# EPOCHDevs/PandasArrow

Hardware: AMD Instinct MI355X
Metric: Grows/sec hash group-by-sum, 1e9 int64 rows x 1e6 keys (higher is better)
Workload: dtype f64; 1 GPU; group_by(int64 key).agg(sum,mean,count), 1e+09 rows / 1e+06 keys, 1 GPU; rows=1000000000, keys=1000000, rows_per_gpu=1000000000, parity=bit-exact vs Arrow-order pairwise sum

## Files before the change

pandasarrow_amd/csrc/gb_flr_reduce.hpp:

```cpp
#pragma once

constexpr int kFlrBits = 6;
constexpr int kFlrLevels = 20;
#ifndef PDX_FLR_ITEMS
#define PDX_FLR_ITEMS 10
#endif
#ifndef PDX_FLR_DENSE_WAVES
#define PDX_FLR_DENSE_WAVES 1
#endif
#ifndef PDX_FLR_BATCH_RANK
#define PDX_FLR_BATCH_RANK 1
#endif
#ifndef PDX_FLR_DPP_SCAN
#define PDX_FLR_DPP_SCAN 1
#endif
constexpr bool kFlrDppScan = PDX_FLR_DPP_SCAN != 0;
#ifndef PDX_FLR_RANK_GROUP
#define PDX_FLR_RANK_GROUP 2
#endif
constexpr int kFlrRankGroup = PDX_FLR_RANK_GROUP;
constexpr bool kFlrBatchRank = PDX_FLR_BATCH_RANK != 0;
constexpr int kFlrDenseWaves = PDX_FLR_DENSE_WAVES;
constexpr int kFlrItems = PDX_FLR_ITEMS;
constexpr int kFlrTile = kSortBlock * kFlrItems;
#ifdef PDX_FLR_TIMING
__device__ unsigned long long g_flr_cycles[2][12];
#define FLR_T(slot)                                                                                     \
  do {                                                                                                  \
    if (DENSE_PW && wave < 2) {                                                                         \
      const unsigned long long now_ = __builtin_readcyclecounter();                                     \
      tacc_[slot] += now_ - tmark_;                                                                     \
      tmark_ = now_;                                                                                    \
    }                                                                                                   \
  } while (0)
#else
#define FLR_T(slot) do { } while (0)
#endif
constexpr int kFlrMaxLeaves = kFlrTile / 16 + ((1 << kFlrBits) * 30) / 16;
constexpr int kFlrLeafStride = kFlrMaxLeaves + 1;
constexpr int kFlrDenseLevels = 16;
__global__ void k_run_starts(const uint32_t* __restrict__ sorted_keys, int64_t n, int low_bits, int64_t nruns, uint32_t* __restrict__ run_start,
                             unsigned int* __restrict__ max_len) {
  const uint32_t lmask = (1u << low_bits) - 1u;
  const int64_t stride = (int64_t)gridDim.x * blockDim.x;
  for (int64_t r = (int64_t)blockIdx.x * blockDim.x + threadIdx.x; r <= nruns; r += stride) {
    int64_t lo = 0, hi = n;
    if (r < nruns) {
      while (lo < hi) {
        int64_t mid = (lo + hi) >> 1;
        if ((int64_t)(sorted_keys[mid] & lmask) < r) lo = mid + 1;
        else hi = mid;
      }
    } else {
      lo = n;
    }
    run_start[r] = (uint32_t)lo;
  }
  (void)max_len;
}
__global__ void k_run_max_len(const uint32_t* __restrict__ run_start, int64_t nruns, unsigned int* __restrict__ out, unsigned int limit) {
  const int64_t stride = (int64_t)gridDim.x * blockDim.x;
  unsigned int m = 0, nl = 0, rl = 0;
  for (int64_t r = (int64_t)blockIdx.x * blockDim.x + threadIdx.x; r < nruns; r += stride) {
    unsigned int len = run_start[r + 1] - run_start[r];
    m = len > m ? len : m;
    if (len > limit) {
      ++nl;
      rl += len;
    }
  }
  for (int d = 32; d >= 1; d >>= 1) {
    unsigned int o = __shfl_xor(m, d, 64);
    m = o > m ? o : m;
// ... 62 lines not shown
    int lo = 0, hi = nl - 1;
    while (lo < hi) {
      const int mid = (lo + hi + 1) >> 1;
      if ((int64_t)soff[mid] <= t) lo = mid;
      else hi = mid - 1;
    }
    const int64_t src = (int64_t)sstart[lo] + (t - (int64_t)soff[lo]);
    const uint32_t k = keys[src];
    uint32_t slot;
    if (sizeof(KT) == 1) slot = (((k & ((1u << kFlrBits) - 1u)) << low_bits) | srun[lo]) | ((k >> 7) << 31);
    else slot = k;
    side_key[t] = slot;
    side_val[t] = vals[src];
  }
}
__device__ __forceinline__ double flr_sqdev(double v, double mu) {
  const double x = v - mu;
  return v != v ? v : (mu != mu ? mu : x * x);
}
__device__ __forceinline__ void flr_counter_push(double (*csum)[1 << kFlrBits], int lane, unsigned long long& cmask, int& root, double leaf) {
  int cur = 0;
  unsigned long long m = 1;
  double v = pw_merge(csum[0][lane], leaf);
  cmask ^= m;
  while ((cmask & m) == 0) {
    csum[cur][lane] = 0.0;
    ++cur;
    m <<= 1;
    v = pw_merge(csum[cur][lane], v);
    cmask ^= m;
  }
  csum[cur][lane] = v;
  root = cur > root ? cur : root;
}
}
#include "flr_wave.hpp"
namespace pdx {
template <int ITEMS, int GROUP>
__device__ __forceinline__ void wave_match_rank_batch(unsigned long long* M, uint32_t* cnt, const uint32_t (&d)[ITEMS], int rows_wave, int lane, uint64_t lt_mask,
                                                      uint32_t (&rank)[ITEMS]) {
#pragma unroll
  for (int q = 0; q < ITEMS; ++q) __hip_atomic_store(&M[q * 64 + lane], 0ull, __ATOMIC_RELAXED, __HIP_MEMORY_SCOPE_WAVEFRONT);
  __builtin_amdgcn_fence(__ATOMIC_ACQ_REL, "wavefront");
#pragma unroll
  for (int q = 0; q < ITEMS; ++q)
    if (q * 64 + lane < rows_wave) __hip_atomic_fetch_or(&M[q * 64 + d[q]], 1ull << lane, __ATOMIC_RELAXED, __HIP_MEMORY_SCOPE_WAVEFRONT);
  __builtin_amdgcn_fence(__ATOMIC_ACQ_REL, "wavefront");
  uint32_t tot = 0;
#pragma unroll
  for (int q0 = 0; q0 < ITEMS; q0 += GROUP) {
    unsigned long long peers[GROUP], own[GROUP];
#pragma unroll
    for (int g = 0; g < GROUP; ++g)
      if (q0 + g < ITEMS) peers[g] = __hip_atomic_load(&M[(q0 + g) * 64 + d[q0 + g]], __ATOMIC_RELAXED, __HIP_MEMORY_SCOPE_WAVEFRONT);
#pragma unroll
    for (int g = 0; g < GROUP; ++g)
      if (q0 + g < ITEMS) own[g] = __hip_atomic_load(&M[(q0 + g) * 64 + lane], __ATOMIC_RELAXED, __HIP_MEMORY_SCOPE_WAVEFRONT);
#pragma unroll
    for (int g = 0; g < GROUP; ++g)
      if (q0 + g < ITEMS) {
        rank[q0 + g] = (uint32_t)__popcll(peers[g] & lt_mask) + (uint32_t)__shfl((int)tot, (int)d[q0 + g], 64);
        tot += (uint32_t)__popcll(own[g]);
      }
  }
  __hip_atomic_store(&cnt[lane], tot, __ATOMIC_RELAXED, __HIP_MEMORY_SCOPE_WAVEFRONT);
  __builtin_amdgcn_fence(__ATOMIC_ACQ_REL, "wavefront");
}
__device__ __forceinline__ uint32_t wave_inclusive_sum_dpp(uint32_t x) {
  x += (uint32_t)__builtin_amdgcn_update_dpp(0, (int)x, 0x111, 0xF, 0xF, true);
  x += (uint32_t)__builtin_amdgcn_update_dpp(0, (int)x, 0x112, 0xF, 0xF, true);
  x += (uint32_t)__builtin_amdgcn_update_dpp(0, (int)x, 0x114, 0xF, 0xF, true);
  x += (uint32_t)__builtin_amdgcn_update_dpp(0, (int)x, 0x118, 0xF, 0xF, true);
  x += (uint32_t)__builtin_amdgcn_update_dpp(0, (int)x, 0x142, 0xA, 0xF, false);
  x += (uint32_t)__builtin_amdgcn_update_dpp(0, (int)x, 0x143, 0xC, 0xF, false);
  return x;
}
struct RunStateOp {
  template <typename U>
  __device__ static U identity() { return U(0); }
  __device__ uint32_t operator()(uint32_t a, uint32_t b) const {
    const uint32_t nh = ((a >> 16) + (b >> 16)) << 16;
    if (b & 0x1000u) return (b & 0xFFFFu) | nh;
    return (((a & 0xFFFu) + (b & 0xFFFu)) & 0xFFFu) | (a & 0x7000u) | nh;
  }
};
template <typename T, bool DENSE_PW, typename KT = uint32_t, bool NULL_PW = false>
__global__ void __launch_bounds__(kSortBlock, (DENSE_PW ? kFlrDenseWaves : 1)) k_flr_reduce(const KT* __restrict__ keys, const T* __restrict__ vals,
                                                           const uint32_t* __restrict__ run_start, int64_t nruns, int low_bits,
                                                           const uint32_t* __restrict__ gid_of_slot, SegOut out, uint8_t* __restrict__ ok,
                                                           int want_pw, int want_mm, int want_is, int nullable,
                                                           const double* __restrict__ sqdev_mean, unsigned int max_run) {
  constexpr int R = 1 << kFlrBits;
  __shared__ __attribute__((aligned(16))) T svals[DENSE_PW ? 16 * kFlrLeafStride : kFlrTile + R];
  __shared__ __attribute__((aligned(8))) uint8_t snull[kFlrTile + R];
  __shared__ uint32_t cnt[kSortWaves][R];
  constexpr bool kBatch = DENSE_PW && kFlrBatchRank;
  static_assert(!kBatch || sizeof(T) * 16 * kFlrLeafStride >= sizeof(unsigned long long) * kSortWaves * kFlrItems * R, "the match words alias the value staging area");
  __shared__ unsigned long long match[kBatch ? 1 : kSortWaves][kBatch ? 1 : R];
  __shared__ uint32_t dstart[R + 1];
  constexpr int kLevels = DENSE_PW ? kFlrDenseLevels : kFlrLevels;
  __shared__ double csum[kLevels][R];
  __shared__ int open_pos[R];
  __shared__ double open_acc[R];
  __shared__ double mu_s[R];
  __shared__ int lp[R + 1];
  __shared__ uint8_t leaf_d[DENSE_PW ? kFlrLeafStride + 3 : 4];
  __shared__ uint32_t dinfo[R];
  __shared__ uint32_t run_smem[8];
  double* leafsum = reinterpret_cast<double*>(snull);
  constexpr bool dense_pw = DENSE_PW;
  const int tid = threadIdx.x, lane = tid & 63, wave = tid >> 6;
  const uint64_t lt_mask = (1ull << lane) - 1ull;
  for (int d = tid; d < kSortWaves * R; d += kSortBlock) {
    (&cnt[0][0])[d] = 0;
    if constexpr (!kBatch) (&match[0][0])[d] = 0;
  }
  __syncthreads();
#ifdef PDX_FLR_TIMING
  unsigned long long tacc_[10] = {};
#endif
  for (int64_t run = blockIdx.x; run < nruns; run += gridDim.x) {
    const int64_t s = run_start[run], e = run_start[run + 1];
    if (s == e || e - s > (int64_t)max_run) continue;
    if (tid < R) {
      open_pos[tid] = 0;
      open_acc[tid] = 0.0;
      mu_s[tid] = 0.0;
    }
    double mu = 0.0;
    bool mu_known = false;
    double acc = 0.0;
    int pos = 0, root = 0;
    int tile_c = 0, tile_lp = 0;
    unsigned long long cmask = 0, isum = 0;
    long long nvalid = 0, nrows = 0;
    T vmn = T(0), vmx = T(0);
    int zneg = -1;
    bool has = false;
    if (wave == 0)
      for (int l = 0; l < kLevels; ++l) csum[l][lane] = 0.0;
    uint32_t key[kFlrItems];
    T val[kFlrItems];
    auto load_tile = [&](int64_t t0) {
      const int rows = (int)(e - t0 < kFlrTile ? e - t0 : kFlrTile);
#pragma unroll
      for (int q = 0; q < kFlrItems; ++q) {
        const int r = wave * (64 * kFlrItems) + q * 64 + lane;
        const int rr = r < rows ? r : rows - 1;
        key[q] = ld_stream<kStreamFlrTile>(keys + t0 + rr);
        val[q] = ld_stream<kStreamFlrTile>(vals + t0 + rr);
      }
    };
    load_tile(s);
#ifdef PDX_FLR_TIMING
    unsigned long long tmark_ = __builtin_readcyclecounter();
#endif
    for (int64_t t0 = s; t0 < e; t0 += kFlrTile) {
      const int rows = (int)(e - t0 < kFlrTile ? e - t0 : kFlrTile);
      uint32_t rank[kFlrItems];
      FLR_T(0);
      if constexpr (kBatch) {
#pragma unroll
        for (int q = 0; q < kFlrItems; ++q) key[q] = sizeof(KT) == 4 ? ((key[q] & kSortKeyMask) >> low_bits) & (R - 1) : key[q] & (R - 1);
        wave_match_rank_batch<kFlrItems, kFlrRankGroup>(reinterpret_cast<unsigned long long*>(svals) + wave * (kFlrItems * R), cnt[wave], key, rows - wave * (64 * kFlrItems), lane,
                                                        lt_mask, rank);
      } else {
#pragma unroll
        for (int q = 0; q < kFlrItems; ++q) {
          const int r = wave * (64 * kFlrItems) + q * 64 + lane;
          const bool active = r < rows;
          const uint32_t d = sizeof(KT) == 4 ? ((key[q] & kSortKeyMask) >> low_bits) & (R - 1) : key[q] & (R - 1);
          rank[q] = wave_match_rank(match[wave], cnt[wave], d, active, lane, lt_mask);
        }
      }
      FLR_T(1);
      __syncthreads();
      FLR_T(2);
      if (tid < R) {
        uint32_t cw[kSortWaves];
#pragma unroll
        for (int w = 0; w < kSortWaves; ++w) cw[w] = cnt[w][tid];
        uint32_t tot = 0;
#pragma unroll
        for (int w = 0; w < kSortWaves; ++w) {
          const uint32_t c = cw[w];
          cw[w] = tot;
          tot += c;
        }
        uint32_t base, inc, ex;
        if (dense_pw) {
          const int c = (int)tot;
          const uint32_t nl = c > 0 ? (uint32_t)(pos + c + 15) >> 4 : 0u;
          const uint32_t both = kFlrDppScan ? wave_inclusive_sum_dpp(tot | (nl << 16)) : wave_inclusive_scan(tot | (nl << 16), SumOp());
          inc = both & 0xFFFFu;
          ex = inc - tot;
          const uint32_t lincl = both >> 16, lex = lincl - nl;
          base = 16u * lex + (uint32_t)pos;
          tile_c = c;
          tile_lp = (int)lex;
          dinfo[tid] = lex | ((uint32_t)pos << 12) | ((uint32_t)c << 16);
          if (c > 0) leaf_d[lex] = (uint8_t)tid;
          if (tid == R - 1) lp[R] = (int)lincl;
          if (sqdev_mean && c > 0 && !mu_known) {
            mu = sqdev_mean[gid_of_slot[((uint32_t)lane << low_bits) | (uint32_t)run]];
            mu_s[lane] = mu;
            mu_known = true;
          }
          nrows += c;
          nvalid += c;
        } else {
          inc = wave_inclusive_scan(tot, SumOp());
          ex = inc - tot;
          base = ex;
          dstart[tid] = ex;
          if (tid == R - 1) dstart[R] = inc;
        }
#pragma unroll
        for (int w = 0; w < kSortWaves; ++w) cnt[w][tid] = cw[w] + base;
        if (NULL_PW) {
          snull[inc + tid] = 2;
          const int c = (int)tot;
          if (sqdev_mean && c > 0 && !mu_known) {
            mu = sqdev_mean[gid_of_slot[((uint32_t)lane << low_bits) | (uint32_t)run]];
            mu_s[lane] = mu;
            mu_known = true;
          }
          nrows += c;
        }
      }
      FLR_T(3);
      __syncthreads();
      FLR_T(4);
#pragma unroll
// ... 35 lines not shown
            const Pair pr = *reinterpret_cast<const Pair*>(svals + e * (2 * kFlrLeafStride) + 2 * Lf);
            xs[2 * e] = seg_to_f64(pr.x);
            xs[2 * e + 1] = seg_to_f64(pr.y);
          }
          const uint32_t di = dinfo[d];
          const double oa = open_acc[d];
          const int j = Lf - (int)(di & 0xFFFu), p0 = (int)((di >> 12) & 15u), c = (int)(di >> 16);
          const int q0 = j == 0 ? p0 : 0;
          int q1 = p0 + c - 16 * j;
          q1 = q1 < 16 ? q1 : 16;
          double a = (j == 0 && p0 > 0) ? oa : 0.0;
          if (sqdev_mean) {
            const double m = mu_s[d];
#pragma unroll
            for (int q = 0; q < 16; ++q)
              if (q >= q0 && q < q1) a += flr_sqdev(xs[q], m);
          } else {
#pragma unroll
            for (int q = 0; q < 16; ++q)
              if (q >= q0 && q < q1) a += xs[q];
          }
          if (a != a) {
            a = (j == 0 && p0 > 0) ? oa : 0.0;
            const double m = sqdev_mean ? mu_s[d] : 0.0;
#pragma unroll
            for (int q = 0; q < 16; ++q)
              if (q >= q0 && q < q1) a = pw_leaf_add(a, sqdev_mean ? flr_sqdev(xs[q], m) : xs[q]);
          }
          leafsum[Lf] = a;
        }
        FLR_T(7);
        __syncthreads();
        FLR_T(8);
        if (wave == 0 && tile_c > 0) {
          const int p0 = pos, c = tile_c;
          const int nl = (p0 + c + 15) >> 4, nfull = (p0 + c) >> 4;
          const double* lf = leafsum + tile_lp;
          const double last = lf[nl - 1];
          if (nfull > 0) {
            double c0 = csum[0][lane], c1 = csum[1][lane], c2 = csum[2][lane];
            double nxt = lf[0];
            for (int j = 0; j < nfull; ++j) {
              double v = nxt;
              if (j + 1 < nfull) nxt = lf[j + 1];
              v = pw_merge(c0, v);
              cmask ^= 1ull;
              if (cmask & 1ull) {
                c0 = v;
              } else {
                c0 = 0.0;
                v = pw_merge(c1, v);
                cmask ^= 2ull;
                if (cmask & 2ull) {
                  c1 = v;
                  root = root > 1 ? root : 1;
                } else {
                  c1 = 0.0;
                  v = pw_merge(c2, v);
                  cmask ^= 4ull;
                  if (cmask & 4ull) {
                    c2 = v;
                    root = root > 2 ? root : 2;
                  } else {
                    c2 = 0.0;
                    int cur = 3;
                    unsigned long long m = 8ull;
                    v = pw_merge(csum[3][lane], v);
                    cmask ^= m;
                    while ((cmask & m) == 0) {
                      csum[cur][lane] = 0.0;
                      ++cur;
                      m <<= 1;
                      v = pw_merge(csum[cur][lane], v);
                      cmask ^= m;
                    }
                    csum[cur][lane] = v;
                    root = cur > root ? cur : root;
                  }
                }
              }
            }
            csum[0][lane] = c0;
            csum[1][lane] = c1;
            csum[2][lane] = c2;
          }
          const int rem = (p0 + c) & 15;
          pos = rem;
          acc = rem ? last : 0.0;
          if (rem) open_acc[lane] = last;
        }
      } else if (NULL_PW) {
        constexpr int CH = (kFlrTile + R + kSortBlock - 1) / kSortBlock;
        const int L = rows + R;
        uint8_t f[CH];
        uint32_t st = 0;
        {
          uint32_t tl = 0, hb = 0, lt = 0, nh = 0;
#pragma unroll
          for (int k = 0; k < CH; ++k) {
            const int pp = tid * CH + k;
            f[k] = pp < L ? snull[pp] : (uint8_t)2;
            if (f[k]) {
              tl = 0;
              hb = 1;
              lt = f[k];
              nh += f[k] == 2;
            } else {
              ++tl;
            }
          }
          st = tl | (hb << 12) | (lt << 13) | (nh << 16);
        }
        uint32_t tot_unused;
// ... 108 lines not shown
            if (ib + u >= i1) break;
            const T x = xb[u];
            const bool isnull = nb[u] != 0;
            bool close = false;
            if (!isnull) {
              ++nvalid;
              if (want_pw) {
                acc = pw_leaf_add(pos == 0 ? 0.0 : acc, sqdev_mean ? flr_sqdev(seg_to_f64(x), mu) : seg_to_f64(x));
                close = ++pos == 16;
              }
              if (want_is) isum += (unsigned long long)x;
              if (want_mm && x == x) {
                if (!has) { vmn = vmx = x; has = true; }
                else {
                  if (x < vmn) vmn = x;
                  if (x > vmx) vmx = x;
                }
                if constexpr (__is_same(T, double)) {
                  if (x == 0.0) zneg = __double_as_longlong(x) < 0 ? 1 : 0;
                }
              }
            } else {
              close = want_pw && pos > 0;
            }
            if (close) {
              reinterpret_cast<double*>(svals)[i0 + nleaf++] = acc;
              pos = 0;
            }
          }
        }
        for (int j = 0; j < nleaf; ++j) flr_counter_push(csum, lane, cmask, root, reinterpret_cast<const double*>(svals)[i0 + j]);
      }
    }
    if (wave == 0 && nrows > 0) {
      const uint32_t slot = ((uint32_t)lane << low_bits) | (uint32_t)run;
      const uint32_t oi = gid_of_slot[slot];
      if (want_pw) {
        if (pos > 0) flr_counter_push(csum, lane, cmask, root, acc);
        double total = 0.0;
        if (nvalid > 0) {
          double a = csum[0][lane];
          for (int i = 1; i <= root; ++i) a = pw_merge(csum[i][lane], a);
          total = a;
        }
        if (out.sum_f) out.sum_f[oi] = total;
        if (out.mean) out.mean[oi] = nvalid ? pw_mean(total, (double)nvalid) : 0.0;
      }
      if (want_is && out.sum_i) out.sum_i[oi] = (long long)isum;
      if (want_mm) {
        T nanv = T(0);
        if constexpr (__is_same(T, double)) nanv = __builtin_nan("");
        if (out.vmin) static_cast<T*>(out.vmin)[oi] = has ? vmn : nanv;
        if constexpr (__is_same(T, double)) {
          if (has && zneg >= 0 && vmx == 0.0 && nvalid < nrows) vmx = zneg ? -0.0 : 0.0;
        }
        if (out.vmax) static_cast<T*>(out.vmax)[oi] = has ? vmx : nanv;
      }
      if (out.count) out.count[oi] = nvalid;
      if (ok) ok[oi] = nvalid > 0;
    }
    __syncthreads();
  }
#ifdef PDX_FLR_TIMING
  if (DENSE_PW && wave < 2 && lane == 0)
    for (int i = 0; i < 10; ++i) atomicAdd(&g_flr_cycles[wave][i], tacc_[i]);
#endif
}
```

pandasarrow_amd/csrc/groupby.hip:

```cpp
#include <stdlib.h>
#include <string.h>
#include <string>
#include <algorithm>
#include <memory>
#include <vector>
#include "compact.hpp"
#include "minmax.hpp"
#include "pairwise.hpp"
#include "radix_sort.hpp"
#include "scan.hpp"
#include "temporal_round.hpp"

namespace pdx {
#include "gb_hash_build.hpp"
#include "gb_dense_slots.hpp"
#include "gb_group_ids.hpp"
#include "gb_seg_reduce.hpp"
#include "gb_resample_kernels.hpp"

}

using namespace pdx;

#include "gb_handle.hpp"
// ... 846 lines not shown
  const int grid = (int)std::min<int64_t>(ceil_div(G, kSegWaves), (int64_t)kCUs * 8);
  if (f64)
    hipLaunchKernelGGL((k_seg_reduce_nullable<double>), dim3(grid), dim3(kSegWaves * 64), 0, st, static_cast<const double*>(vals), flag_keys, row_valid,
                       valid_off, seg_start, G, oidx, oo, ok_bytes);
  else
    hipLaunchKernelGGL((k_seg_reduce_nullable<long long>), dim3(grid), dim3(kSegWaves * 64), 0, st, static_cast<const long long*>(vals), flag_keys,
                       row_valid, valid_off, seg_start, G, oidx, oo, ok_bytes);
  PDX_LAUNCH_CHECK();
  return reduce_huge_nullable_groups(vals, f64 ? PDX_FLOAT64 : PDX_INT64, flag_keys, row_valid, valid_off, seg_start, G, oidx, n, oo, ok_bytes, s, st);
}
static int reduce_full(const pdx_groupby* gb, const GroupedLayout& L, const void* vals, bool f64, const SegOut& oo, bool pw, bool mm, bool is,
                       const uint32_t* oidx, uint8_t* ok_bytes, Scratch& s, hipStream_t st) {
  return reduce_segments(L.validity != nullptr, L.flag_keys, L.row_valid, L.offset, L.seg_start, gb->G, gb->n, vals, f64, oo, pw, mm, is, oidx, ok_bytes, s, st);
}
static int reduce_side(const pdx_groupby* gb, const GroupedLayout& L, const SegOut& oo, bool pw, bool mm, bool is, uint8_t* ok_bytes, const double* sqmean,
                       Scratch& s, hipStream_t st) {
  const bool is_f = L.dtype == PDX_FLOAT64, nullable = L.validity != nullptr;
  const void* vals = L.side_vals;
  bool f64 = is_f;
  if (sqmean) {
    double* d = s.get<double>((size_t)L.side_rows);
    PDX_SCRATCH_CHECK(s);
    PDX_PROFILE("seg_sqdev", st);
    const int grid = (int)std::min<int64_t>(ceil_div(gb->G, 4), (int64_t)kCUs * 16);
    if (is_f) hipLaunchKernelGGL((k_seg_sqdev<double>), dim3(grid), dim3(256), 0, st, reinterpret_cast<const double*>(L.side_vals), L.side_seg, gb->G, sqmean, d, gb->gid_of_occ);
    else hipLaunchKernelGGL((k_seg_sqdev<long long>), dim3(grid), dim3(256), 0, st, reinterpret_cast<const long long*>(L.side_vals), L.side_seg, gb->G, sqmean, d, gb->gid_of_occ);
    PDX_LAUNCH_CHECK();
    vals = d;
    f64 = true;
  }
  return reduce_segments(nullable, L.side_keys, nullptr, 0, L.side_seg, gb->G, L.side_rows, vals, f64, oo, pw, mm, is, gb->gid_of_occ, ok_bytes, s, st);
}

static int reduce_fused(const pdx_groupby* gb, const GroupedLayout& L, const AggTuning& t, const SegOut& oo, bool pw, bool mm, bool is, uint8_t* okbytes,
                        const double* sqmean, Scratch& s, hipStream_t st, std::string* reducer) {
  if (L.side_rows) PDX_TRY(reduce_side(gb, L, oo, pw, mm, is, okbytes, sqmean, s, st));
  const unsigned int max_run = L.max_run ? L.max_run : 0xFFFFFFFFu;
  PDX_PROFILE("fused_last_digit_reduce", st);
  const bool nullable = L.validity != nullptr, is_f = L.dtype == PDX_FLOAT64;
  const int64_t nruns = L.nruns, n = gb->n;
  const int low_bits = L.low_bits;
  const uint8_t* keys8 = L.keys8;
  const uint32_t* keys_sorted = L.fkeys;
  const uint64_t* vs = L.fvals;
  const uint32_t* run_start = L.run_start;
  const int grid = (int)std::min<int64_t>(nruns, (int64_t)kCUs * t.flr_wgs_per_cu);
  const bool dense = pw && !mm && !is && !nullable;
  const bool nullpw = pw && !mm && !is && nullable && t.null_pw;
#define FLR_LAUNCH(TT, DD)                                                                                                                       \
  if (keys8 && nullpw)                                                                                                                           \
    hipLaunchKernelGGL((k_flr_reduce<TT, false, uint8_t, true>), dim3(grid), dim3(kSortBlock), 0, st, keys8, reinterpret_cast<const TT*>(vs), run_start, \
                       nruns, low_bits, gb->gid_of_slot, oo, okbytes, (int)pw, (int)mm, (int)is, 1, sqmean, max_run);                              \
  else if (nullpw)                                                                                                                               \
    hipLaunchKernelGGL((k_flr_reduce<TT, false, uint32_t, true>), dim3(grid), dim3(kSortBlock), 0, st, keys_sorted, reinterpret_cast<const TT*>(vs),   \
                       run_start, nruns, low_bits, gb->gid_of_slot, oo, okbytes, (int)pw, (int)mm, (int)is, 1, sqmean, max_run);                   \
  else if (keys8)                                                                                                                                \
    hipLaunchKernelGGL((k_flr_reduce<TT, DD, uint8_t>), dim3(grid), dim3(kSortBlock), 0, st, keys8, reinterpret_cast<const TT*>(vs), run_start, nruns, \
                       low_bits, gb->gid_of_slot, oo, okbytes, (int)pw, (int)mm, (int)is, nullable ? 1 : 0, sqmean, max_run);                      \
  else                                                                                                                                           \
    hipLaunchKernelGGL((k_flr_reduce<TT, DD>), dim3(grid), dim3(kSortBlock), 0, st, keys_sorted, reinterpret_cast<const TT*>(vs), run_start, nruns, \
                       low_bits, gb->gid_of_slot, oo, okbytes, (int)pw, (int)mm, (int)is, nullable ? 1 : 0, sqmean, max_run)
  const bool wave_form = !nullpw && (t.wave_force >= 0 ? t.wave_force != 0 : !dense);
  if (reducer) *reducer = wave_form ? "flr_wave" : (nullpw ? "flr_reduce_nullpw" : (dense ? "flr_reduce_dense" : "flr_reduce"));
  if (wave_form) {
    const int wgrid = (int)std::min<int64_t>(nruns, (int64_t)kCUs * t.fw_wgs_per_cu);
    const bool pw_only = pw && !mm && !is;
    const uint64_t max_leaves = nullable ? (uint64_t)L.hmax + 1 : (uint64_t)L.hmax / 16 + 2;
    const int fw_levels = std::max(2, ilog2(max_leaves + 1));
    const size_t fw_lds = (size_t)fw_lds_bytes(nullable, fw_levels);
#define FW_LAUNCH(TT, KK, KPTR, NN, PP)                                                                                                  \
  hipLaunchKernelGGL((k_flr_wave<TT, KK, NN, PP>), dim3(wgrid), dim3(64), fw_lds, st, KPTR, reinterpret_cast<const TT*>(vs), n, run_start, nruns, low_bits, \
                     gb->gid_of_slot, oo, okbytes, (int)pw, (int)mm, (int)is, sqmean, fw_levels, max_run)
#define FW_DISPATCH(TT)                                                                        \
  if (keys8) {                                                                                 \
    if (nullable) { if (pw_only) FW_LAUNCH(TT, uint8_t, keys8, true, true); else FW_LAUNCH(TT, uint8_t, keys8, true, false); }          \
    else { if (pw_only) FW_LAUNCH(TT, uint8_t, keys8, false, true); else FW_LAUNCH(TT, uint8_t, keys8, false, false); }              \
  } else {                                                                                     \
    if (nullable) { if (pw_only) FW_LAUNCH(TT, uint32_t, keys_sorted, true, true); else FW_LAUNCH(TT, uint32_t, keys_sorted, true, false); } \
    else { if (pw_only) FW_LAUNCH(TT, uint32_t, keys_sorted, false, true); else FW_LAUNCH(TT, uint32_t, keys_sorted, false, false); } \
  }
    if (is_f) { FW_DISPATCH(double) } else { FW_DISPATCH(long long) }
#undef FW_DISPATCH
#undef FW_LAUNCH
  } else if (is_f) {
    if (dense) { FLR_LAUNCH(double, true); }
    else { FLR_LAUNCH(double, false); }
  } else {
    if (dense) { FLR_LAUNCH(long long, true); }
    else { FLR_LAUNCH(long long, false); }
  }
#undef FLR_LAUNCH
  PDX_LAUNCH_CHECK();
  return PDX_OK;
}

__global__ void k_mean_from_cache(const double* __restrict__ sum, const long long* __restrict__ cnt, int64_t G, double* __restrict__ out) {
  int64_t stride = (int64_t)gridDim.x * blockDim.x;
  for (int64_t i = (int64_t)blockIdx.x * blockDim.x + threadIdx.x; i < G; i += stride) out[i] = cnt[i] ? pw_mean(sum[i], (double)cnt[i]) : 0.0;
}

static GroupedLayout* find_bound(pdx_groupby* gb, const pdx_column* values) {
  const void* vv = validity_or_null(values);
  for (auto& b : gb->bound)
    if (b->values == values->values && b->offset == values->offset && b->dtype == values->dtype && b->validity == vv) {
      b->last_use = ++gb->use_clock;
      return b.get();
    }
  return nullptr;
}
static size_t bind_limit_bytes(const pdx_groupby* gb) {
  if (gb->bind_limit) return gb->bind_limit;
  if (const char* e = getenv("PDX_BIND_MAX_BYTES")) return (size_t)atoll(e);
  size_t free_b = 0, total_b = 0;
  if (hipMemGetInfo(&free_b, &total_b) != hipSuccess) {
    (void)hipGetLastError();
    return (size_t)64 << 30;
  }
  return total_b / 4;
}
static void enforce_bind_limit(pdx_groupby* gb, const GroupedLayout* keep) {
  const size_t limit = bind_limit_bytes(gb);
  for (;;) {
    size_t total = 0;
    for (auto& b : gb->bound) total += b->bytes;
// ... 100 lines not shown
      case PDX_AGG_MAX: want_dt = values->dtype; o.vmax = oc->values; rq.want_mm = true; rq.want_std5 = true; break;
      case PDX_AGG_COUNT: want_dt = PDX_INT64; o.count = static_cast<long long*>(oc->values); needs_validity = false; rq.want_std5 = true; break;
      case PDX_AGG_VARIANCE: want_dt = PDX_FLOAT64; rq.var_out = static_cast<double*>(oc->values); break;
      case PDX_AGG_STDDEV: want_dt = PDX_FLOAT64; rq.std_out = static_cast<double*>(oc->values); break;
      case PDX_AGG_PRODUCT: want_dt = values->dtype; rq.prod_out = oc->values; break;
      case PDX_AGG_FIRST: want_dt = values->dtype; rq.first_out = oc->values; break;
      case PDX_AGG_LAST: want_dt = values->dtype; rq.last_out = oc->values; break;
      default: return fail(PDX_INVALID, "pdx_groupby_agg: unknown aggregate kind");
    }
    if (oc->dtype != want_dt) return fail(PDX_INVALID, "pdx_groupby_agg: output dtype does not match the aggregate's result type");
    if (needs_validity && !oc->validity)
      return fail(PDX_INVALID, "pdx_groupby_agg: values carry nulls but an output has no validity buffer");
    oc->length = G;
    oc->null_count = needs_validity ? -1 : 0;
  }
  if (G == 0) return PDX_OK;
  const AggTuning t = AggTuning::read();
  GroupedLayout local;
  GroupedLayout* Lp = find_bound(gb, values);
  const bool bound = Lp != nullptr;
  if (!Lp) Lp = &local;
  GroupedLayout& L = *Lp;
  const bool std_only = rq.std_only();
  const size_t bytes_before = L.bytes;
  const AccTuning at = AccTuning::read();
  const bool order_free = rq.want_std5 && !rq.want_pw && !rq.var_out && !rq.std_out && !rq.prod_out && !rq.first_out && !rq.last_out;
  AccGeom ag;
  if (order_free && !(bound && rq.want_is) && !L.fused && !L.full)
    ag = acc_geometry(gb, vvalid != nullptr, (o.vmin ? kAccMin : 0u) | (o.vmax ? kAccMax : 0u) | (o.sum_i ? kAccSum : 0u) | (o.count ? kAccCnt : 0u), is_f, at);
  const bool use_acc = ag.ok;
  if (!use_acc && ((!L.fused && !L.full) || (!std_only && !L.full))) PDX_TRY(build_layout(gb, values, std_only, t, L, st));
  const bool use_fused = std_only && L.fused;
  Scratch s;
  std::string reducer, acc_plan;
  auto pack_validity = [&](uint8_t* bits, const uint8_t* ok_bytes) {
    if (!bits) return;
    if (!ok_bytes) hipMemsetAsync(bits, 0xFF, (size_t)((G + 7) / 8), st);
    else hipLaunchKernelGGL(k_pack_bytes, dim3(grid_for((G + 7) / 8, 256)), dim3(256), 0, st, ok_bytes, G, bits);
  };
  auto reduce_std = [&](const SegOut& oo, bool pw, bool mm, bool is, uint8_t* okb) -> int {
    if (use_acc) {
      reducer = "lds_acc";
      return reduce_acc(gb, ag, values, oo, okb, at, s, st, &acc_plan);
    }
    if (use_fused) return reduce_fused(gb, L, t, oo, pw, mm, is, okb, nullptr, s, st, &reducer);
    reducer = vvalid ? "seg_reduce_nullable" : "seg_reduce";
    return reduce_full(gb, L, L.vals_sorted, is_f, oo, pw, mm, is, L.out_index, okb, s, st);
  };
  std::string cache_note;
  if (rq.want_std5 && bound) {
    const bool have_cnt = L.have_pw || L.have_count, have_isum = L.have_pw || L.have_is;
    const bool need_sumfam = (rq.want_pw && !L.have_pw) || (rq.want_is && !have_isum) || (o.count && !have_cnt), need_mm = rq.want_mm && !L.have_mm;
    if (use_acc && (need_sumfam || need_mm)) {
      const bool need_is = rq.want_is && !have_isum, need_cnt = o.count && !have_cnt;
      if (need_cnt && !L.c_count) L.c_count = L.own<long long>((size_t)G);
      if (vvalid && !L.c_ok) L.c_ok = L.own<uint8_t>((size_t)G);
      if (need_is && !L.c_isum) L.c_isum = L.own<long long>((size_t)G);
      if (need_mm && !L.c_min) {
        L.c_min = L.own<uint64_t>((size_t)G);
        L.c_max = L.own<uint64_t>((size_t)G);
      }
      if ((need_cnt && !L.c_count) || (vvalid && !L.c_ok) || (need_is && !L.c_isum) || (need_mm && (!L.c_min || !L.c_max))) return PDX_OOM;
      SegOut c{};
      if (need_cnt) c.count = L.c_count;
      if (need_is) c.sum_i = L.c_isum;
      if (need_mm) {
        c.vmin = L.c_min;
        c.vmax = L.c_max;
      }
      PDX_TRY(reduce_std(c, false, need_mm, need_is, L.c_ok));
      L.have_count = L.have_count || need_cnt;
      L.have_is = L.have_is || need_is;
      L.have_mm = L.have_mm || need_mm;
      cache_note = " cache=fill";
    } else if (need_sumfam || need_mm) {
      if (!L.c_count) L.c_count = L.own<long long>((size_t)G);
      if (vvalid && !L.c_ok) L.c_ok = L.own<uint8_t>((size_t)G);
      if (need_sumfam && !L.c_sum) L.c_sum = L.own<double>((size_t)G);
// ... 22 lines not shown
      reducer = "none";
    }
    const size_t gb8 = (size_t)G * 8;
    if (o.sum_f) PDX_HIP(hipMemcpyAsync(o.sum_f, L.c_sum, gb8, hipMemcpyDeviceToDevice, st));
    if (o.sum_i) PDX_HIP(hipMemcpyAsync(o.sum_i, L.c_isum, gb8, hipMemcpyDeviceToDevice, st));
    if (o.count) PDX_HIP(hipMemcpyAsync(o.count, L.c_count, gb8, hipMemcpyDeviceToDevice, st));
    if (o.vmin) PDX_HIP(hipMemcpyAsync(o.vmin, L.c_min, gb8, hipMemcpyDeviceToDevice, st));
    if (o.vmax) PDX_HIP(hipMemcpyAsync(o.vmax, L.c_max, gb8, hipMemcpyDeviceToDevice, st));
    if (o.mean) hipLaunchKernelGGL(k_mean_from_cache, dim3(grid_for(G, 256)), dim3(256), 0, st, L.c_sum, L.c_count, G, o.mean);
    for (int k = 0; k < nk; ++k)
      if (kinds[k] <= PDX_AGG_COUNT) pack_validity(static_cast<uint8_t*>(outs[k].validity), kinds[k] == PDX_AGG_COUNT ? nullptr : L.c_ok);
    PDX_LAUNCH_CHECK();
  } else if (rq.want_std5) {
    uint8_t* okb = vvalid ? s.get<uint8_t>((size_t)G) : nullptr;
    PDX_SCRATCH_CHECK(s);
    PDX_TRY(reduce_std(o, rq.want_pw, rq.want_mm, rq.want_is, okb));
    for (int k = 0; k < nk; ++k)
      if (kinds[k] <= PDX_AGG_COUNT) pack_validity(static_cast<uint8_t*>(outs[k].validity), kinds[k] == PDX_AGG_COUNT ? nullptr : okb);
    PDX_LAUNCH_CHECK();
  }
  if (rq.var_out || rq.std_out) {
    double* m2 = s.get<double>((size_t)G);
    long long* cnt_g = s.get<long long>((size_t)G);
    uint8_t* ok2 = vvalid ? s.get<uint8_t>((size_t)G) : nullptr;
    uint8_t* ok1 = vvalid ? s.get<uint8_t>((size_t)G) : nullptr;
    double* mean_g = s.get<double>((size_t)G);
    PDX_SCRATCH_CHECK(s);
    SegOut o1{};
    o1.mean = mean_g;
    SegOut o2{};
    o2.sum_f = m2;
    o2.count = cnt_g;
    if (use_fused) {
      PDX_TRY(reduce_fused(gb, L, t, o1, true, false, false, ok1, nullptr, s, st, &reducer));
      PDX_TRY(reduce_fused(gb, L, t, o2, true, false, false, ok2, mean_g, s, st, nullptr));
    } else {
      if (reducer.empty()) reducer = vvalid ? "seg_reduce_nullable" : "seg_reduce";
      double* d = s.get<double>((size_t)n);
      PDX_SCRATCH_CHECK(s);
      PDX_TRY(reduce_full(gb, L, L.vals_sorted, is_f, o1, true, false, false, nullptr, ok1, s, st));
      {
        PDX_PROFILE("seg_sqdev", st);
        const int grid = (int)std::min<int64_t>(ceil_div(G, 4), (int64_t)kCUs * 16);
        if (is_f) hipLaunchKernelGGL((k_seg_sqdev<double>), dim3(grid), dim3(256), 0, st, static_cast<const double*>(L.vals_sorted), L.seg_start, G, mean_g, d);
        else hipLaunchKernelGGL((k_seg_sqdev<long long>), dim3(grid), dim3(256), 0, st, static_cast<const long long*>(L.vals_sorted), L.seg_start, G, mean_g, d);
        PDX_LAUNCH_CHECK();
      }
      PDX_TRY(reduce_full(gb, L, d, true, o2, true, false, false, L.out_index, ok2, s, st));
    }
    hipLaunchKernelGGL(k_var_finish, dim3(grid_for(G, 256)), dim3(256), 0, st, m2, cnt_g, G, rq.var_out, rq.std_out);
    for (int k = 0; k < nk; ++k)
      if (kinds[k] == PDX_AGG_VARIANCE || kinds[k] == PDX_AGG_STDDEV) pack_validity(static_cast<uint8_t*>(outs[k].validity), ok2);
    PDX_LAUNCH_CHECK();
  }
  if (rq.prod_out || rq.first_out || rq.last_out) {
    uint8_t* pok = (vvalid && rq.prod_out) ? s.get<uint8_t>((size_t)G) : nullptr;
    uint8_t* fok = (vvalid && rq.first_out) ? s.get<uint8_t>((size_t)G) : nullptr;
    uint8_t* lok = (vvalid && rq.last_out) ? s.get<uint8_t>((size_t)G) : nullptr;
    PDX_SCRATCH_CHECK(s);
    {
      PDX_PROFILE("seg_product_first_last", st);
      const int pf_grid = (int)std::min<int64_t>(ceil_div(G, 4), (int64_t)kCUs * 16);
      if (is_f)
        hipLaunchKernelGGL((k_seg_product_first_last<double>), dim3(pf_grid), dim3(256), 0, st, static_cast<const double*>(L.vals_sorted), L.flag_keys,
                           L.row_valid, values->offset, L.seg_start, G, L.out_index, static_cast<double*>(rq.prod_out), pok, static_cast<double*>(rq.first_out),
                           fok, static_cast<double*>(rq.last_out), lok);
      else
        hipLaunchKernelGGL((k_seg_product_first_last<long long>), dim3(pf_grid), dim3(256), 0, st, static_cast<const long long*>(L.vals_sorted),
// ... 247 lines not shown
```

Before: 70.69 Grows/s.

## Defer deep pairwise-counter carries and flatten low-level push into branchless selects

Reworks the wave-0 binary-counter pairwise summation loop. The low three levels are now updated with branchless merges and selects. Carries into levels 3 and up are held in a pending value and inserted later through a batched, wave-uniform deep-insert routine that loads four levels at a time. The aim is to cut lane divergence and serialized shared-memory loops in the per-leaf push. The cost is extra speculative pw_merge work on every step and more complex carry logic that must keep the merge order bit-exact.

After: 71.13 Grows/s (median of 6 runs). No clear change (+0.6%).

```diff
diff --git a/pandasarrow_amd/csrc/gb_flr_reduce.hpp b/pandasarrow_amd/csrc/gb_flr_reduce.hpp
--- a/pandasarrow_amd/csrc/gb_flr_reduce.hpp
+++ b/pandasarrow_amd/csrc/gb_flr_reduce.hpp
@@ -18,6 +18,14 @@
 #ifndef PDX_FLR_RANK_GROUP
 #define PDX_FLR_RANK_GROUP 2
 #endif
+#ifndef PDX_FLR_DEFER_DEEP
+#define PDX_FLR_DEFER_DEEP 1
+#endif
+constexpr bool kFlrDeferDeep = PDX_FLR_DEFER_DEEP != 0;
+#ifndef PDX_FLR_FLAT_PUSH
+#define PDX_FLR_FLAT_PUSH 1
+#endif
+constexpr bool kFlrFlatPush = PDX_FLR_FLAT_PUSH != 0 && kFlrDeferDeep;
 constexpr int kFlrRankGroup = PDX_FLR_RANK_GROUP;
 constexpr bool kFlrBatchRank = PDX_FLR_BATCH_RANK != 0;
 constexpr int kFlrDenseWaves = PDX_FLR_DENSE_WAVES;
@@ -167,6 +175,26 @@
   }
   csum[cur][lane] = v;
   root = cur > root ? cur : root;
+}
+template <int LEVELS>
+__device__ __forceinline__ void flr_deep_insert(double (*csum)[1 << kFlrBits], int lane, unsigned long long& cmask, int& root, double v) {
+  const int land = 3 + __ffs((int)~(uint32_t)(cmask >> 3)) - 1;
+  for (int base = 3;; base += 4) {
+    double a[4];
+#pragma unroll
+    for (int i = 0; i < 4; ++i) a[i] = csum[base + i < LEVELS ? base + i : LEVELS - 1][lane];
+#pragma unroll
+    for (int i = 0; i < 4; ++i) {
+      const int l = base + i;
+      if (l <= land) {
+        v = pw_merge(a[i], v);
+        csum[l < LEVELS ? l : LEVELS - 1][lane] = l < land ? 0.0 : v;
+      }
+    }
+    if (__ballot(land > base + 3) == 0ull) break;
+  }
+  cmask += 8ull;
+  root = land > root ? land : root;
 }
 }
 #include "flr_wave.hpp"
@@ -252,7 +280,7 @@
   }
   __syncthreads();
 #ifdef PDX_FLR_TIMING
-  unsigned long long tacc_[10] = {};
+  unsigned long long tacc_[12] = {};
 #endif
   for (int64_t run = blockIdx.x; run < nruns; run += gridDim.x) {
     const int64_t s = run_start[run], e = run_start[run + 1];
@@ -443,9 +471,32 @@
           if (nfull > 0) {
             double c0 = csum[0][lane], c1 = csum[1][lane], c2 = csum[2][lane];
             double nxt = lf[0];
+            double pend = 0.0;
+            bool pending = false;
+            FLR_T(11);
+            const bool crowded = kFlrDeferDeep && __ballot(nfull > 8) != 0ull;
             for (int j = 0; j < nfull; ++j) {
               double v = nxt;
               if (j + 1 < nfull) nxt = lf[j + 1];
+              if constexpr (kFlrFlatPush) {
+                const uint32_t lo = (uint32_t)cmask & 7u;
+                const bool b0 = (lo & 1u) != 0, b01 = (lo & 3u) == 3u, b012 = lo == 7u;
+                const double s0 = pw_merge(c0, v);
+                const double s1 = pw_merge(c1, s0);
+                const double s2 = pw_merge(c2, s1);
+                if (crowded) {
+                  if (b012 && pending) flr_deep_insert<kLevels>(csum, lane, cmask, root, pend);
+                }
+                c2 = b01 ? (b012 ? 0.0 : s2) : c2;
+                c1 = b0 ? (b01 ? 0.0 : s1) : c1;
+                c0 = b0 ? 0.0 : s0;
+                pend = b012 ? s2 : pend;
+                pending = pending || b012;
+                const int land = b01 ? 2 : (b0 ? 1 : 0);
+                root = (!b012 && land > root) ? land : root;
+                cmask = (cmask & ~7ull) | (unsigned long long)((lo + 1u) & 7u);
+                continue;
+              }
               v = pw_merge(c0, v);
               cmask ^= 1ull;
               if (cmask & 1ull) {
@@ -466,22 +517,33 @@
                     root = root > 2 ? root : 2;
                   } else {
                     c2 = 0.0;
-                    int cur = 3;
-                    unsigned long long m = 8ull;
-                    v = pw_merge(csum[3][lane], v);
-                    cmask ^= m;
-                    while ((cmask & m) == 0) {
-                      csum[cur][lane] = 0.0;
-                      ++cur;
-                      m <<= 1;
-                      v = pw_merge(csum[cur][lane], v);
+                    if constexpr (kFlrDeferDeep) {
+                      if (crowded && pending) flr_deep_insert<kLevels>(csum, lane, cmask, root, pend);
+                      pend = v;
+                      pending = true;
+                    } else {
+                      int cur = 3;
+                      unsigned long long m = 8ull;
+                      v = pw_merge(csum[3][lane], v);
                       cmask ^= m;
+                      while ((cmask & m) == 0) {
+                        csum[cur][lane] = 0.0;
+                        ++cur;
+                        m <<= 1;
+                        v = pw_merge(csum[cur][lane], v);
+                        cmask ^= m;
+                      }
+                      csum[cur][lane] = v;
+                      root = cur > root ? cur : root;
                     }
-                    csum[cur][lane] = v;
-                    root = cur > root ? cur : root;
                   }
                 }
               }
+            }
+            if constexpr (kFlrDeferDeep) {
+              FLR_T(0);
+              if (pending) flr_deep_insert<kLevels>(csum, lane, cmask, root, pend);
+              FLR_T(10);
             }
             csum[0][lane] = c0;
             csum[1][lane] = c1;
@@ -687,6 +749,6 @@
   }
 #ifdef PDX_FLR_TIMING
   if (DENSE_PW && wave < 2 && lane == 0)
-    for (int i = 0; i < 10; ++i) atomicAdd(&g_flr_cycles[wave][i], tacc_[i]);
-#endif
-}
+    for (int i = 0; i < 12; ++i) atomicAdd(&g_flr_cycles[wave][i], tacc_[i]);
+#endif
+}
```

## Split fused last-digit reduce: stream leaf sums to global, build pairwise trees in second kernel

Applied to the files above, without the earlier changes.

In the dense pairwise path, the fused reducer no longer runs the per-group pairwise counter tree in LDS. Each tile's 16-row leaf sums and per-digit descriptors are written to a global handoff buffer. A new k_flr_trees kernel then has one wave per run combine those leaves, keeping the low tree levels in registers, to produce sum, mean and count. This removes the serial wave-0 tree work and the large csum LDS array from the streaming kernel. The cost is extra global traffic for leaves and descriptors, a second kernel launch, and more scratch memory.

New measurement: 69.71 Grows/s before, 70.04 Grows/s after, median of 6. Within noise of the previous version (+0.5%).

```diff
diff --git a/pandasarrow_amd/csrc/gb_flr_reduce.hpp b/pandasarrow_amd/csrc/gb_flr_reduce.hpp
--- a/pandasarrow_amd/csrc/gb_flr_reduce.hpp
+++ b/pandasarrow_amd/csrc/gb_flr_reduce.hpp
@@ -14,6 +14,10 @@
 #ifndef PDX_FLR_DPP_SCAN
 #define PDX_FLR_DPP_SCAN 1
 #endif
+#ifndef PDX_FLR_HANDOFF
+#define PDX_FLR_HANDOFF 1
+#endif
+constexpr bool kFlrHandoff = PDX_FLR_HANDOFF != 0;
 constexpr bool kFlrDppScan = PDX_FLR_DPP_SCAN != 0;
 #ifndef PDX_FLR_RANK_GROUP
 #define PDX_FLR_RANK_GROUP 2
@@ -39,6 +43,9 @@
 constexpr int kFlrMaxLeaves = kFlrTile / 16 + ((1 << kFlrBits) * 30) / 16;
 constexpr int kFlrLeafStride = kFlrMaxLeaves + 1;
 constexpr int kFlrDenseLevels = 16;
+__host__ __device__ constexpr int64_t flr_handoff_slot(int64_t s, int64_t run, int64_t k) { return s / kFlrTile + run + k; }
+constexpr int64_t flr_handoff_slots(int64_t n, int64_t nruns) { return n / kFlrTile + nruns + 1; }
+static_assert(kFlrMaxLeaves <= kFlrLeafStride && kFlrMaxLeaves < (1 << 12) && kFlrTile < (1 << 16), "a tile's leaves fit a slot, and first leaf | rows fit a descriptor word");
 __global__ void k_run_starts(const uint32_t* __restrict__ sorted_keys, int64_t n, int low_bits, int64_t nruns, uint32_t* __restrict__ run_start,
                              unsigned int* __restrict__ max_len) {
   const uint32_t lmask = (1u << low_bits) - 1u;
@@ -224,7 +231,8 @@
                                                            const uint32_t* __restrict__ run_start, int64_t nruns, int low_bits,
                                                            const uint32_t* __restrict__ gid_of_slot, SegOut out, uint8_t* __restrict__ ok,
                                                            int want_pw, int want_mm, int want_is, int nullable,
-                                                           const double* __restrict__ sqdev_mean, unsigned int max_run) {
+                                                           const double* __restrict__ sqdev_mean, unsigned int max_run,
+                                                           double* __restrict__ leafbuf, uint32_t* __restrict__ descbuf) {
   constexpr int R = 1 << kFlrBits;
   __shared__ __attribute__((aligned(16))) T svals[DENSE_PW ? 16 * kFlrLeafStride : kFlrTile + R];
   __shared__ __attribute__((aligned(8))) uint8_t snull[kFlrTile + R];
@@ -233,8 +241,9 @@
   static_assert(!kBatch || sizeof(T) * 16 * kFlrLeafStride >= sizeof(unsigned long long) * kSortWaves * kFlrItems * R, "the match words alias the value staging area");
   __shared__ unsigned long long match[kBatch ? 1 : kSortWaves][kBatch ? 1 : R];
   __shared__ uint32_t dstart[R + 1];
+  constexpr bool kHand = DENSE_PW && kFlrHandoff;
   constexpr int kLevels = DENSE_PW ? kFlrDenseLevels : kFlrLevels;
-  __shared__ double csum[kLevels][R];
+  __shared__ double csum[kHand ? 1 : kLevels][R];
   __shared__ int open_pos[R];
   __shared__ double open_acc[R];
   __shared__ double mu_s[R];
@@ -254,6 +263,14 @@
 #ifdef PDX_FLR_TIMING
   unsigned long long tacc_[10] = {};
 #endif
+  int64_t pend_slot = 0;
+  int pend_nl = 0;
+  auto publish_leaves = [&]() {
+    if constexpr (kHand) {
+      for (int Lf = tid; Lf < pend_nl; Lf += kSortBlock) leafbuf[pend_slot * kFlrLeafStride + Lf] = leafsum[Lf];
+      pend_nl = 0;
+    }
+  };
   for (int64_t run = blockIdx.x; run < nruns; run += gridDim.x) {
     const int64_t s = run_start[run], e = run_start[run + 1];
     if (s == e || e - s > (int64_t)max_run) continue;
@@ -272,8 +289,10 @@
     T vmn = T(0), vmx = T(0);
     int zneg = -1;
     bool has = false;
-    if (wave == 0)
-      for (int l = 0; l < kLevels; ++l) csum[l][lane] = 0.0;
+    if constexpr (!kHand)
+      if (wave == 0)
+        for (int l = 0; l < kLevels; ++l) csum[l][lane] = 0.0;
+    int64_t hslot = flr_handoff_slot(s, run, 0);
     uint32_t key[kFlrItems];
     T val[kFlrItems];
     auto load_tile = [&](int64_t t0) {
@@ -309,6 +328,7 @@
         }
       }
       FLR_T(1);
+      publish_leaves();
       __syncthreads();
       FLR_T(2);
       if (tid < R) {
@@ -334,6 +354,7 @@
           tile_c = c;
           tile_lp = (int)lex;
           dinfo[tid] = lex | ((uint32_t)pos << 12) | ((uint32_t)c << 16);
+          if constexpr (kHand) descbuf[hslot * R + tid] = lex | ((uint32_t)pos << 12) | ((uint32_t)c << 16);
           if (c > 0) leaf_d[lex] = (uint8_t)tid;
           if (tid == R - 1) lp[R] = (int)lincl;
           if (sqdev_mean && c > 0 && !mu_known) {
@@ -435,7 +456,15 @@
         FLR_T(7);
         __syncthreads();
         FLR_T(8);
-        if (wave == 0 && tile_c > 0) {
+        if constexpr (kHand) {
+          if (wave == 0 && tile_c > 0) {
+            const int nl = (pos + tile_c + 15) >> 4, rem = (pos + tile_c) & 15;
+            if (rem) open_acc[lane] = leafsum[tile_lp + nl - 1];
+            pos = rem;
+          }
+          pend_slot = hslot++;
+          pend_nl = NL;
+        } else if (wave == 0 && tile_c > 0) {
           const int p0 = pos, c = tile_c;
           const int nl = (p0 + c + 15) >> 4, nfull = (p0 + c) >> 4;
           const double* lf = leafsum + tile_lp;
@@ -656,7 +685,7 @@
         for (int j = 0; j < nleaf; ++j) flr_counter_push(csum, lane, cmask, root, reinterpret_cast<const double*>(svals)[i0 + j]);
       }
     }
-    if (wave == 0 && nrows > 0) {
+    if (!kHand && wave == 0 && nrows > 0) {
       const uint32_t slot = ((uint32_t)lane << low_bits) | (uint32_t)run;
       const uint32_t oi = gid_of_slot[slot];
       if (want_pw) {
@@ -685,8 +714,129 @@
     }
     __syncthreads();
   }
+  publish_leaves();
 #ifdef PDX_FLR_TIMING
   if (DENSE_PW && wave < 2 && lane == 0)
     for (int i = 0; i < 10; ++i) atomicAdd(&g_flr_cycles[wave][i], tacc_[i]);
 #endif
 }
+
+constexpr int kFlrTreeWaves = 4;
+constexpr int kFlrTreeAhead = 4;
+constexpr int kFlrTreeRegLevels = 3;
+constexpr size_t flr_trees_lds_bytes(int levels) { return sizeof(double) * kFlrTreeWaves * (size_t)(levels - kFlrTreeRegLevels) * (1 << kFlrBits); }
+__global__ void __launch_bounds__(kFlrTreeWaves * 64, 8) k_flr_trees(const uint32_t* __restrict__ run_start, int64_t nruns, int low_bits,
+                                                                  const uint32_t* __restrict__ gid_of_slot, SegOut out, uint8_t* __restrict__ ok,
+                                                                  const double* __restrict__ leafbuf, const uint32_t* __restrict__ descbuf,
+                                                                  unsigned int max_run, int levels) {
+  constexpr int R = 1 << kFlrBits;
+  extern __shared__ double flr_trees_lds[];
+  const int lane = threadIdx.x & 63, wave = threadIdx.x >> 6;
+  const int64_t run = (int64_t)blockIdx.x * kFlrTreeWaves + wave;
+  if (run >= nruns) return;
+  const int64_t s = run_start[run], e = run_start[run + 1];
+  if (s == e || e - s > (int64_t)max_run) return;
+  double(*csum)[R] = reinterpret_cast<double(*)[R]>(flr_trees_lds) + wave * (levels - kFlrTreeRegLevels) - kFlrTreeRegLevels;
+  for (int l = kFlrTreeRegLevels; l < levels; ++l) csum[l][lane] = 0.0;
+  double c0 = 0.0, c1 = 0.0, c2 = 0.0;
+  unsigned long long cmask = 0;
+  int root = 0;
+  auto push = [&](double v) {
+    v = pw_merge(c0, v);
+    cmask ^= 1ull;
+    if (cmask & 1ull) {
+      c0 = v;
+      return;
+    }
+    c0 = 0.0;
+    v = pw_merge(c1, v);
+    cmask ^= 2ull;
+    if (cmask & 2ull) {
+      c1 = v;
+      root = root > 1 ? root : 1;
+      return;
+    }
+    c1 = 0.0;
+    v = pw_merge(c2, v);
+    cmask ^= 4ull;
+    if (cmask & 4ull) {
+      c2 = v;
+      root = root > 2 ? root : 2;
+      return;
+    }
+    c2 = 0.0;
+    int cur = 3;
+    unsigned long long m = 8ull;
+    v = pw_merge(csum[3][lane], v);
+    cmask ^= m;
+    while ((cmask & m) == 0) {
+      csum[cur][lane] = 0.0;
+      ++cur;
+      m <<= 1;
+      v = pw_merge(csum[cur][lane], v);
+      cmask ^= m;
+    }
+    csum[cur][lane] = v;
+    root = cur > root ? cur : root;
+  };
+  const int ntiles = (int)((e - s + kFlrTile - 1) / kFlrTile);
+  const int64_t slot0 = flr_handoff_slot(s, run, 0);
+  const uint32_t* dp = descbuf + slot0 * R + lane;
+  const double* lb = leafbuf + slot0 * kFlrLeafStride;
+  struct Tile {
+    const double* lf;
+    int nfull, rem, c;
+    double pre[kFlrTreeAhead], last;
+  };
+  auto request = [&](uint32_t d, int k) {
+    Tile t;
+    const int lex = (int)(d & 0xFFFu), p0 = (int)((d >> 12) & 15u);
+    t.c = (int)(d >> 16);
+    t.lf = lb + (int64_t)k * kFlrLeafStride + lex;
+    t.nfull = (p0 + t.c) >> 4;
+    t.rem = (p0 + t.c) & 15;
+    t.last = 0.0;
+#pragma unroll
+    for (int j = 0; j < kFlrTreeAhead; ++j) t.pre[j] = j < t.nfull ? t.lf[j] : 0.0;
+    if (t.c > 0 && t.rem) t.last = t.lf[t.nfull];
+    return t;
+  };
+  uint32_t d1 = ntiles > 1 ? dp[R] : 0u;
+  Tile cur = request(dp[0], 0);
+  double acc = 0.0;
+  int pos = 0;
+  long long nrows = 0;
+  for (int k = 0; k < ntiles; ++k) {
+    const uint32_t d2 = k + 2 < ntiles ? dp[(int64_t)(k + 2) * R] : 0u;
+    Tile nxt = cur;
+    if (k + 1 < ntiles) nxt = request(d1, k + 1);
+    d1 = d2;
+    if (cur.c > 0) {
+#pragma unroll
+      for (int j = 0; j < kFlrTreeAhead; ++j)
+        if (j < cur.nfull) push(cur.pre[j]);
+      if (cur.nfull > kFlrTreeAhead) {
+        double nx = cur.lf[kFlrTreeAhead];
+        for (int j = kFlrTreeAhead; j < cur.nfull; ++j) {
+          const double v = nx;
+          if (j + 1 < cur.nfull) nx = cur.lf[j + 1];
+          push(v);
+        }
+      }
+      pos = cur.rem;
+      acc = cur.rem ? cur.last : 0.0;
+      nrows += cur.c;
+    }
+    cur = nxt;
+  }
+  if (nrows > 0) {
+    const uint32_t oi = gid_of_slot[((uint32_t)lane << low_bits) | (uint32_t)run];
+    if (pos > 0) push(acc);
+    double a = c0;
+    for (int i = 1; i <= root; ++i) a = pw_merge(i == 1 ? c1 : (i == 2 ? c2 : csum[i][lane]), a);
+    if (out.sum_f) out.sum_f[oi] = a;
+    if (out.mean) out.mean[oi] = pw_mean(a, (double)nrows);
+    if (out.count) out.count[oi] = nrows;
+    if (ok) ok[oi] = 1;
+  }
+}
diff --git a/pandasarrow_amd/csrc/groupby.hip b/pandasarrow_amd/csrc/groupby.hip
--- a/pandasarrow_amd/csrc/groupby.hip
+++ b/pandasarrow_amd/csrc/groupby.hip
@@ -902,8 +902,12 @@
   return reduce_segments(nullable, L.side_keys, nullptr, 0, L.side_seg, gb->G, L.side_rows, vals, f64, oo, pw, mm, is, gb->gid_of_occ, ok_bytes, s, st);
 }
 
+struct FlrHandoff {
+  double* leaf = nullptr;
+  uint32_t* desc = nullptr;
+};
 static int reduce_fused(const pdx_groupby* gb, const GroupedLayout& L, const AggTuning& t, const SegOut& oo, bool pw, bool mm, bool is, uint8_t* okbytes,
-                        const double* sqmean, Scratch& s, hipStream_t st, std::string* reducer) {
+                        const double* sqmean, Scratch& s, FlrHandoff& ho, hipStream_t st, std::string* reducer) {
   if (L.side_rows) PDX_TRY(reduce_side(gb, L, oo, pw, mm, is, okbytes, sqmean, s, st));
   const unsigned int max_run = L.max_run ? L.max_run : 0xFFFFFFFFu;
   PDX_PROFILE("fused_last_digit_reduce", st);
@@ -920,18 +924,25 @@
 #define FLR_LAUNCH(TT, DD)                                                                                                                       \
   if (keys8 && nullpw)                                                                                                                           \
     hipLaunchKernelGGL((k_flr_reduce<TT, false, uint8_t, true>), dim3(grid), dim3(kSortBlock), 0, st, keys8, reinterpret_cast<const TT*>(vs), run_start, \
-                       nruns, low_bits, gb->gid_of_slot, oo, okbytes, (int)pw, (int)mm, (int)is, 1, sqmean, max_run);                              \
+                       nruns, low_bits, gb->gid_of_slot, oo, okbytes, (int)pw, (int)mm, (int)is, 1, sqmean, max_run, nullptr, nullptr);            \
   else if (nullpw)                                                                                                                               \
     hipLaunchKernelGGL((k_flr_reduce<TT, false, uint32_t, true>), dim3(grid), dim3(kSortBlock), 0, st, keys_sorted, reinterpret_cast<const TT*>(vs),   \
-                       run_start, nruns, low_bits, gb->gid_of_slot, oo, okbytes, (int)pw, (int)mm, (int)is, 1, sqmean, max_run);                   \
+                       run_start, nruns, low_bits, gb->gid_of_slot, oo, okbytes, (int)pw, (int)mm, (int)is, 1, sqmean, max_run, nullptr, nullptr); \
   else if (keys8)                                                                                                                                \
     hipLaunchKernelGGL((k_flr_reduce<TT, DD, uint8_t>), dim3(grid), dim3(kSortBlock), 0, st, keys8, reinterpret_cast<const TT*>(vs), run_start, nruns, \
-                       low_bits, gb->gid_of_slot, oo, okbytes, (int)pw, (int)mm, (int)is, nullable ? 1 : 0, sqmean, max_run);                      \
+                       low_bits, gb->gid_of_slot, oo, okbytes, (int)pw, (int)mm, (int)is, nullable ? 1 : 0, sqmean, max_run, ho.leaf, ho.desc);    \
   else                                                                                                                                           \
     hipLaunchKernelGGL((k_flr_reduce<TT, DD>), dim3(grid), dim3(kSortBlock), 0, st, keys_sorted, reinterpret_cast<const TT*>(vs), run_start, nruns, \
-                       low_bits, gb->gid_of_slot, oo, okbytes, (int)pw, (int)mm, (int)is, nullable ? 1 : 0, sqmean, max_run)
+                       low_bits, gb->gid_of_slot, oo, okbytes, (int)pw, (int)mm, (int)is, nullable ? 1 : 0, sqmean, max_run, ho.leaf, ho.desc)
   const bool wave_form = !nullpw && (t.wave_force >= 0 ? t.wave_force != 0 : !dense);
   if (reducer) *reducer = wave_form ? "flr_wave" : (nullpw ? "flr_reduce_nullpw" : (dense ? "flr_reduce_dense" : "flr_reduce"));
+  const bool handoff = kFlrHandoff && dense && !wave_form;
+  if (handoff && !ho.leaf) {
+    const int64_t slots = flr_handoff_slots(n, nruns);
+    ho.leaf = s.get<double>((size_t)slots * kFlrLeafStride);
+    ho.desc = s.get<uint32_t>((size_t)slots << kFlrBits);
+    PDX_SCRATCH_CHECK(s);
+  }
   if (wave_form) {
     const int wgrid = (int)std::min<int64_t>(nruns, (int64_t)kCUs * t.fw_wgs_per_cu);
     const bool pw_only = pw && !mm && !is;
@@ -960,6 +971,11 @@
     else { FLR_LAUNCH(long long, false); }
   }
 #undef FLR_LAUNCH
+  if (handoff) {
+    const int levels = std::min(kFlrDenseLevels, std::max(kFlrTreeRegLevels + 1, ilog2((uint64_t)L.hmax / 16 + 3)));
+    hipLaunchKernelGGL(k_flr_trees, dim3((unsigned)ceil_div(nruns, (int64_t)kFlrTreeWaves)), dim3(kFlrTreeWaves * 64), flr_trees_lds_bytes(levels), st, run_start,
+                       nruns, low_bits, gb->gid_of_slot, oo, okbytes, ho.leaf, ho.desc, max_run, levels);
+  }
   PDX_LAUNCH_CHECK();
   return PDX_OK;
 }
@@ -1126,6 +1142,7 @@
   if (!use_acc && ((!L.fused && !L.full) || (!std_only && !L.full))) PDX_TRY(build_layout(gb, values, std_only, t, L, st));
   const bool use_fused = std_only && L.fused;
   Scratch s;
+  FlrHandoff ho;
   std::string reducer, acc_plan;
   auto pack_validity = [&](uint8_t* bits, const uint8_t* ok_bytes) {
     if (!bits) return;
@@ -1137,7 +1154,7 @@
       reducer = "lds_acc";
       return reduce_acc(gb, ag, values, oo, okb, at, s, st, &acc_plan);
     }
-    if (use_fused) return reduce_fused(gb, L, t, oo, pw, mm, is, okb, nullptr, s, st, &reducer);
+    if (use_fused) return reduce_fused(gb, L, t, oo, pw, mm, is, okb, nullptr, s, ho, st, &reducer);
     reducer = vvalid ? "seg_reduce_nullable" : "seg_reduce";
     return reduce_full(gb, L, L.vals_sorted, is_f, oo, pw, mm, is, L.out_index, okb, s, st);
   };
@@ -1226,8 +1243,8 @@
     o2.sum_f = m2;
     o2.count = cnt_g;
     if (use_fused) {
-      PDX_TRY(reduce_fused(gb, L, t, o1, true, false, false, ok1, nullptr, s, st, &reducer));
-      PDX_TRY(reduce_fused(gb, L, t, o2, true, false, false, ok2, mean_g, s, st, nullptr));
+      PDX_TRY(reduce_fused(gb, L, t, o1, true, false, false, ok1, nullptr, s, ho, st, &reducer));
+      PDX_TRY(reduce_fused(gb, L, t, o2, true, false, false, ok2, mean_g, s, ho, st, nullptr));
     } else {
       if (reducer.empty()) reducer = vvalid ? "seg_reduce_nullable" : "seg_reduce";
       double* d = s.get<double>((size_t)n);
```
